# gmlwns2000/sea-attention

Hardware: AMD Instinct MI355X
Metric: tokens/sec + achieved HBM GB/s, OPT-1.3B SEA T=4096 k=64, 1/2/4/8 MI355X (higher is better)
Workload: dtype bf16

## Files before the change

include/sea_hip.h:

```cpp
#ifndef SEA_HIP_H
#define SEA_HIP_H

#include <stdint.h>

#ifdef __cplusplus
extern "C" {
#endif

#define SEA_ABI_VERSION 6

enum sea_dtype { SEA_F32 = 0, SEA_F16 = 1, SEA_BF16 = 2 };

enum sea_error {
  SEA_OK = 0,
  SEA_EINVAL = -1,
  SEA_EUNSUPPORTED = -2,
  SEA_ELAUNCH = -3
};

typedef void* sea_stream_t;

int sea_version(void);
const char* sea_last_error(void);

// ... 42 lines not shown

int sea_csr_elmul(const float* in_values, float* out_values,
                  const void* other, int dtype, const int64_t* other_strides ,
                  int64_t N, int64_t H, int64_t T_dst, int64_t T_src,
                  const void* crow, const void* col, int idx_bytes, int64_t col_stride_n,
                  sea_stream_t stream);

int sea_csr_spmm(const float* values, const void* v, int dtype,
                 int64_t N, int64_t H, int64_t T_dst, int64_t T_src, int64_t D,
                 const int64_t* v_strides ,
                 const void* crow, const void* col, int idx_bytes, int64_t col_stride_n,
                 const int32_t* head_off,
                 float* out, sea_stream_t stream);

enum sea_attn_path { SEA_ATTN_AUTO = 0, SEA_ATTN_GATHER = 1, SEA_ATTN_TILE = 2, SEA_ATTN_KEYRANGE = 3 };
enum { SEA_ATTN_ROW_POOL_SHIFT = 4 };
int sea_sparse_attention(const void* q, const void* k, const void* v, int dtype,
                         int64_t N, int64_t H, int64_t T_dst, int64_t T_src, int64_t D,
                         const int64_t* q_strides, const int64_t* k_strides, const int64_t* v_strides,
                         const int32_t* crow, const int32_t* col, int64_t col_stride_n,
                         const int32_t* head_off,
                         const float* row_scale,
                         const void* avg, const int64_t* avg_strides,
                         const float* mix,
                         void* out, int out_dtype, const int64_t* out_strides,
                         float* probs_out, int64_t probs_stride_n,
                         const uint8_t* block_path,
                         int flags,
                         const uint32_t* bits, int64_t T_m, int is_causal, int max_k, int write_cols,
                         const int32_t* t_src_dev,
                         int64_t t_src_stride,
// ... 120 lines not shown
```

sea-attention_amd/_lib.py:

```python
import ctypes
import os
from ctypes import c_int, c_int32, c_int64, c_void_p, c_char_p, POINTER

import torch

from . import _build

SEA_F32, SEA_F16, SEA_BF16 = 0, 1, 2
ABI_VERSION = 6
_DTYPES = {torch.float32: SEA_F32, torch.float16: SEA_F16, torch.bfloat16: SEA_BF16}

_lib = None

i64 = c_int64
ptr = c_void_p
_i64p = POINTER(c_int64)

_SIGNATURES = {
    "sea_version": ([], c_int),
    "sea_last_error": ([], c_char_p),
    "sea_topk_select": ([ptr, c_int, i64, i64, i64, i64, i64, i64, i64, ptr, i64, i64, c_int, c_int,
                         ptr, ptr, ptr, ptr, ptr], c_int),
    "sea_mask_to_bits": ([ptr, c_int, i64, i64, i64, i64, i64, i64, i64, i64, c_int, c_int,
                          ptr, ptr, ptr, ptr], c_int),
# ... 47 lines not shown
                                ptr, i64, ptr, i64, i64, ptr, i64, ptr, i64, ptr, ptr, ptr, i64, c_int32, c_int32, c_int32, ptr],
                               c_int),
    "sea_performer_avg_supported": ([i64, i64, c_int], c_int),
    "sea_performer_plan": ([i64, i64, i64, i64, i64, c_int, _i64p, _i64p], c_int),
}

EXPORTED_SYMBOLS = tuple(_SIGNATURES)


def library_path():
    return _build.LIB_PATH


SEA_ATTN_AUTO, SEA_ATTN_GATHER, SEA_ATTN_TILE, SEA_ATTN_KEYRANGE = 0, 1, 2, 3
SEA_ATTN_ROW_POOL_SHIFT = 4
SEA_OK, SEA_EINVAL, SEA_EUNSUPPORTED = 0, -1, -2


def load(build_if_missing=True):
    global _lib
    if _lib is not None:
        return _lib
    override = os.environ.get("SEA_HIP_LIB")
    if override:
        if not os.path.exists(override):
            raise RuntimeError(f"SEA_HIP_LIB={override} does not exist")
        path = override
    else:
        path = _build.LIB_PATH
        if _build.is_stale():
# ... 92 lines not shown
```

sea-attention_amd/csrc/sea_attn.hip:

```cpp
#include "sea_attn.hpp"

namespace sea {

template <typename T, typename TO, int LPR, int U, bool WP>
__global__ __launch_bounds__(256) void sparse_attn_kernel(AttnParams p) {
  constexpr int VEC = Elem<T>::VEC;
  constexpr int KPI = 64 / LPR;
  int pair, tb;
  if (!map_block(p.N * p.H, p.TB, &pair, &tb)) return;
  const int n = pair / p.H, h = pair - n * p.H;
  const int t = tb * 4 + (threadIdx.x >> 6);
  if (t >= p.T_dst) return;
  if (kernel_is_idle(p)) return;
  const int lane = threadIdx.x & 63;
  const int grp = lane / LPR, sub = lane - grp * LPR;
  const bool dact = sub * VEC < p.D;

  const T* qp = reinterpret_cast<const T*>(p.q) + n * p.qs[0] + h * p.qs[1] + t * p.qs[2] + sub * VEC;
  const T* kb = reinterpret_cast<const T*>(p.k) + n * p.ks[0] + h * p.ks[1] + sub * VEC;
  const T* vb = reinterpret_cast<const T*>(p.v) + n * p.vs[0] + h * p.vs[1] + sub * VEC;

  uint4 qraw = make_uint4(0, 0, 0, 0);
  if (dact) qraw = *reinterpret_cast<const uint4*>(qp);
  const int row_beg = p.crow[(int64_t)n * (p.T_dst + 1) + t];
// ... 238 lines not shown
  return col[ec];
}

constexpr int SEA_ATTN_WARM_ROWS = 8;

template <typename T, typename TO, int LPR, int U, bool WP, int NWB, bool FUSE, bool DEC, bool ORD, bool X80>
__device__ __forceinline__ void attn_rows_body(const AttnParams& p) {
  static_assert(!DEC || FUSE, "the decode form is a fused form");
  static_assert(!ORD || (FUSE && !DEC && !WP), "rows are dealt from pools in the fused inference form only");
  static_assert(!X80 || LPR == 8, "d = 80: eight lanes per row");
  using F = RowFrag<T, X80>;
  constexpr int VEC = F::VEC, NF = F::NF;
  constexpr int RPW = 64 / LPR;
  constexpr int RPB = NWB * RPW;
  int pair, tb;
  if (kernel_is_idle(p) || !map_block(p.N * p.H, p.TB, &pair, &tb)) return;
  const int n = pair / p.H;
  const int h = (pair - n * p.H + n) % p.H;
  const int lane = threadIdx.x & 63;
  const int grp = lane / LPR, sub = lane - grp * LPR;
  const int gi = (int)(threadIdx.x >> 6) * RPW + grp;
  bool rowok;
  int t;
  if constexpr (ORD) {
    if (!pooled_row<LPR, RPB>(p, n, h, tb, grp, &t, &rowok)) return;
  } else {
    t = tb * RPB + rows_by_length<LPR, RPB>(slot_length(p, n, h, tb * RPB + gi), gi, sub, &rowok);
  }
  const bool dact = X80 || sub * VEC < p.D;
  const int tt = t < p.T_dst ? t : p.T_dst - 1;
  const int sube = dact ? sub : 0;
// ... 86 lines not shown
        }
        softmax_step<U>(s, mnew, vr, m, l, acc);
      }
    }
  }

  const int64_t ridx = ((int64_t)n * p.H + h) * p.T_dst + t;
  if (WP && rowok) {
    const float c = attn_row_factor(p, ridx, l);
    float* pr = p.probs + n * p.probs_stride_n;
    for (int e = beg + sub; e < end; e += LPR) pr[e] = __expf(pr[e] - m) * c;
  }
  if (rowok && dact) attn_epilogue<T, TO, X80>(p, ridx, n, h, t, sub, l, acc);
}

template <typename T, typename TO, int LPR, int U, bool WP, int NWB = 4, bool FUSE = false, bool DEC = false, bool ORD = false>
__global__ __launch_bounds__(NWB * 64, (FUSE && !DEC && sizeof(T) == 2 && !WP) ? 8 : 1) void sparse_attn_rows_kernel(AttnParams p) {
  attn_rows_body<T, TO, LPR, U, WP, NWB, FUSE, DEC, ORD, false>(p);
}

template <typename T, typename TO, int U, bool WP, int NWB = 4, bool FUSE = false, bool DEC = false, bool ORD = false>
__global__ __launch_bounds__(NWB * 64) void sparse_attn_rows80_kernel(AttnParams p) {
  attn_rows_body<T, TO, 8, U, WP, NWB, FUSE, DEC, ORD, true>(p);
}

template <int LPR, bool X80>
struct Decode1Lds {
  static constexpr int CH = LPR == 8 ? 256 : 128;
  static constexpr int DL = LPR * (8 + (X80 ? 2 : 0));
  static constexpr int bytes = CH * 8 + CH + CH * DL * 2;
};

template <typename T, typename TO, int LPR, bool X80 = false, bool PAGED = false, bool WP = false>
// ... 481 lines not shown
    const int64_t pool = 1ll << pool_log2;
    SEA_REQUIRE(pool <= 1024, SEA_EUNSUPPORTED, "%s: %s takes pools of at most 1024 rows (got %lld)", nm, rp, (long long)pool);
    const int64_t rpb = (dtype == SEA_F32 ? D > 32 : (D > 64 && D != 80)) ? 32 : 64;
    SEA_REQUIRE(pool % rpb == 0, SEA_EUNSUPPORTED, "%s: %s needs a pool that is a multiple of the %lld rows of a workgroup (got %lld)",
                nm, rp, (long long)rpb, (long long)pool);
    const int64_t pools = (T_dst + pool - 1) / pool, need = H * pools * pool;
    SEA_REQUIRE(block_path != nullptr && aligned16(block_path) && probs_stride_n >= need, SEA_EINVAL,
                "%s: %s needs a 16-byte aligned uint16 workspace in block_path with probs_stride_n >= %lld elements per batch "
                "item (got %lld)", nm, rp, (long long)need, (long long)probs_stride_n);
    order = reinterpret_cast<const uint16_t*>(block_path);
    order_stride_n = probs_stride_n;
    block_path = nullptr;
    probs_stride_n = 0;
  }
  const bool keyrange = (flags & 0xff) == SEA_ATTN_KEYRANGE;
  KeyRangeParams kr = {nullptr, 0, 0, 0};
  if (keyrange) {
    SEA_REQUIRE(bits != nullptr, SEA_EUNSUPPORTED, "%s: the key-range form is a fused form (bits is NULL)", nm);
    SEA_REQUIRE(t_src_dev == nullptr && block_table == nullptr && t_src_stride == 0, SEA_EUNSUPPORTED,
                "%s: the key-range form has no decode or paged form (t_src_dev / block_table)", nm);
    SEA_REQUIRE(write_cols == 0, SEA_EUNSUPPORTED, "%s: the key-range form writes no columns (write_cols must be 0)", nm);
    SEA_REQUIRE(N > 0 && H > 0 && T_dst > 0 && T_src > 0 && D > 0, SEA_EINVAL, "%s: bad shape", nm);
    SEA_REQUIRE(dtype == SEA_F32 ? (D == 32 || D == 64) : (D == 64 || D == 128), SEA_EUNSUPPORTED,
                "%s: the key-range form takes 16-bit D in {64, 128} or fp32 D in {32, 64} (dtype %d, D=%lld)", nm, dtype, (long long)D);
    const int64_t rk = (flags >> 16) & 0x7fff;
    SEA_REQUIRE(rk > 0, SEA_EINVAL, "%s: the key-range form needs range_keys (1 .. 32767) in bits 16..30 of flags", nm);
    const int64_t nr = (T_src + rk - 1) / rk;
    SEA_REQUIRE(nr <= 64, SEA_EUNSUPPORTED, "%s: the key-range form takes at most 64 ranges (%lld keys in ranges of %lld: %lld)", nm,
                (long long)T_src, (long long)rk, (long long)nr);
    SEA_REQUIRE(block_path == nullptr, SEA_EINVAL, "%s: the key-range form takes no plan (block_path must be NULL)", nm);
// ... 59 lines not shown
  p.probs = probs_out; p.probs_stride_n = probs_stride_n;
  p.sel = nullptr; p.sel_want = 0; p.TB16 = (int)((T_dst + 15) / 16);
  p.sel_count = nullptr; p.sel_total = (int)(N * H * p.TB16);
  p.sel_num = D >= 128 ? 13 : 1; p.sel_den = D >= 128 ? 20 : 2;
  p.bits = bits; p.col_w = const_cast<int32_t*>(col); p.T_m = (int)T_m; p.W = (int)((H * T_m + 31) / 32);
  p.max_k = max_k; p.is_causal = is_causal;
  p.fuse_cap = 8192;
  p.write_cols = write_cols != 0;
  p.t_src_dev = t_src_dev;
  SEA_REQUIRE(t_src_stride >= 0 && t_src_stride * N < (1ll << 31), SEA_EINVAL, "%s: bad T_src stride %lld", nm,
              (long long)t_src_stride);
  p.t_src_stride = (int)t_src_stride;
  p.table = block_table; p.table_stride = (int)table_stride; p.page_shift = block_table ? __builtin_ctzll(page_rows) : 0;
  p.order = order; p.order_stride_n = order_stride_n;
  p.pool_rows = order ? 1 << pool_log2 : 0; p.pools = order ? (int)((T_dst + p.pool_rows - 1) / p.pool_rows) : 0;
  if (t_src_dev) {
    SEA_REQUIRE(bits != nullptr && T_dst <= SEA_ATTN_WARM_ROWS, SEA_EUNSUPPORTED,
                "%s: the decode form takes T_dst <= %d rows per sequence", nm, SEA_ATTN_WARM_ROWS);
    SEA_REQUIRE(probs_out == nullptr || probs_stride_n >= col_stride_n, SEA_EINVAL,
                "%s: the decode form's probs_out needs probs_stride_n >= col_stride_n (%lld < %lld)", nm,
                (long long)probs_stride_n, (long long)col_stride_n);
  }
  if (bits) {
    SEA_REQUIRE(path != SEA_ATTN_TILE && block_path == nullptr, SEA_EUNSUPPORTED, "%s: the fused interpolation runs on the gather kernels", nm);
    SEA_REQUIRE(T_m > 0 && T_m % 32 == 0 && max_k > 0, SEA_EUNSUPPORTED, "%s: fused interpolation needs T_m %% 32 == 0", nm);
    if (t_src_dev) SEA_REQUIRE(H * T_src < (1ll << 31), SEA_EUNSUPPORTED, "%s: the decode form needs int32 ids (H*T_cap < 2^31)", nm);
    else SEA_REQUIRE(H * T_src < (1ll << 24), SEA_EUNSUPPORTED, "%s: H*T_src must stay below 2^24 (fp32-exact ids)", nm);
  }
  p.TB = (int)((T_dst + 3) / 4);
  hipStream_t s = (hipStream_t)stream;
// ... 20 lines not shown
    p.sel_want = 1;
    rc = launch_attn_tile(p, dtype, out_dtype, flags, s);
    SEA_REQUIRE(rc == SEA_OK, rc, "%s: tile kernel launch parameters rejected (flags 0x%x)", nm, flags);
    SEA_CHECK_LAUNCH(nm);
    p.sel_want = 0;
  }
  if (dtype == SEA_F32) rc = launch_attn<float, float>(p, s);
  else if (dtype == SEA_F16) rc = out_dtype == SEA_F32 ? launch_attn<__half, float>(p, s) : launch_attn<__half, __half>(p, s);
  else rc = out_dtype == SEA_F32 ? launch_attn<__hip_bfloat16, float>(p, s) : launch_attn<__hip_bfloat16, __hip_bfloat16>(p, s);
  SEA_REQUIRE(rc == SEA_OK, rc, "%s: unsupported head size %lld", nm, (long long)D);
  SEA_CHECK_LAUNCH(nm);
  return SEA_OK;
}

extern "C" int64_t sea_attention_few_rows(void) { return SEA_ATTN_FEW_ROWS; }

extern "C" int sea_attention_plan(const uint32_t* bits, int64_t N, int64_t H, int64_t T_dst, int64_t T_src, int64_t T_m,
                                  int is_causal, float entries_per_tile, uint8_t* block_path, sea_stream_t stream) {
  const char* nm = "sea_attention_plan";
  SEA_REQUIRE(bits && block_path, SEA_EINVAL, "%s: null pointer", nm);
  SEA_REQUIRE(N > 0 && H > 0 && T_dst > 0 && T_src > 0 && T_m > 0, SEA_EINVAL, "%s: bad shape", nm);
  SEA_REQUIRE(hipMemsetAsync(block_path + plan_count_offset(N, H, (T_dst + 15) / 16), 0, 4, (hipStream_t)stream) == hipSuccess,
              SEA_ELAUNCH, "%s: memset failed", nm);
  const int rc = launch_attn_plan(bits, (int)N, (int)H, (int)T_dst, (int)T_src, (int)T_m, is_causal,
                                  entries_per_tile > 0.f ? entries_per_tile : 30.0f, block_path, (hipStream_t)stream);
  SEA_REQUIRE(rc == SEA_OK, rc, "%s: needs T_m %% 32 == 0, H <= 64 and H * T_m <= 32768", nm);
  SEA_CHECK_LAUNCH(nm);
  return SEA_OK;
}

// ... 70 lines not shown
```

sea-attention_amd/csrc/sea_attn.hpp:

```cpp
#pragma once
#include "sea_common.hpp"

namespace sea {

struct AttnParams {
  const void *q, *k, *v;
  int64_t qs[3], ks[3], vs[3];
  int N, H, T_dst, T_src, D;
  const int32_t* crow;
  const int32_t* col;
  int64_t col_stride_n;
  const int32_t* head_off;
  const float* row_scale;
  const void* avg;
  int64_t as[3];
  const float* mix;
  void* out;
  int64_t os[3];
  float* probs;
  int64_t probs_stride_n;
  const uint8_t* sel;
  int sel_want, TB16;
  const int32_t* sel_count;
  int sel_total, sel_num, sel_den;
  int TB;
  const uint32_t* bits;
  int32_t* col_w;
  int T_m, W, max_k, is_causal, fuse_cap;
  int write_cols;
  const int32_t* t_src_dev;
  int t_src_stride;
  const int32_t* table;
  int table_stride, page_shift;
  const uint16_t* order;
  int64_t order_stride_n;
  int pool_rows, pools;
};

template <typename TO, int VEC> __device__ inline void store_frag(TO* dst, const float* f);
template <> __device__ inline void store_frag<float, 4>(float* dst, const float* f) {
  *reinterpret_cast<float4*>(dst) = make_float4(f[0], f[1], f[2], f[3]);
}
template <> __device__ inline void store_frag<float, 8>(float* dst, const float* f) {
  *reinterpret_cast<float4*>(dst) = make_float4(f[0], f[1], f[2], f[3]);
  *reinterpret_cast<float4*>(dst + 4) = make_float4(f[4], f[5], f[6], f[7]);
}
template <> __device__ inline void store_frag<__hip_bfloat16, 8>(__hip_bfloat16* dst, const float* f) {
  union { uint4 u; __hip_bfloat16 h[8]; } r;
#pragma unroll
  for (int i = 0; i < 8; ++i) r.h[i] = __float2bfloat16(f[i]);
  *reinterpret_cast<uint4*>(dst) = r.u;
// ... 5 lines not shown
  *reinterpret_cast<uint4*>(dst) = r.u;
}
template <> __device__ inline void store_frag<__hip_bfloat16, 4>(__hip_bfloat16* dst, const float* f) {
  union { uint2 u; __hip_bfloat16 h[4]; } r;
#pragma unroll
  for (int i = 0; i < 4; ++i) r.h[i] = __float2bfloat16(f[i]);
  *reinterpret_cast<uint2*>(dst) = r.u;
}
template <> __device__ inline void store_frag<__half, 4>(__half* dst, const float* f) {
  union { uint2 u; __half h[4]; } r;
#pragma unroll
  for (int i = 0; i < 4; ++i) r.h[i] = __float2half(f[i]);
  *reinterpret_cast<uint2*>(dst) = r.u;
}

__device__ inline bool map_block(int NH, int TB, int* pair, int* tb) {
  const int bid = blockIdx.x;
  const int xcd = bid & 7, slot = bid >> 3;
  const int pl = slot / TB;
  const int full = NH >> 3;
  if (pl < full) {
    *tb = slot - pl * TB;
    *pair = pl * 8 + xcd;
    return true;
  }
  const int r = NH - full * 8;
  const int item = (slot - pl * TB) * 8 + xcd;
  if (pl > full || item >= r * TB) return false;
  const int pr = item / TB;
  *tb = item - pr * TB;
  *pair = full * 8 + pr;
  return true;
}

template <int CTRL> __device__ inline float dpp_f(float x) {
  return __int_as_float(__builtin_amdgcn_update_dpp(0, __float_as_int(x), CTRL, 0xF, 0xF, true));
}

template <int LPR> __device__ inline float group_sum(float x) {
  if (LPR >= 2) x += dpp_f<0xB1>(x);
  if (LPR >= 4) x += dpp_f<0x4E>(x);
  if (LPR >= 8) x += dpp_f<0x141>(x);
  if (LPR >= 16) x += dpp_f<0x140>(x);
  if (LPR >= 32) x += __shfl_xor(x, 16);
  if (LPR >= 64) x += __shfl_xor(x, 32);
  return x;
}
// ... 195 lines not shown
```

sea-attention_amd/csrc/sea_attn_tile.hip:

```cpp
#include "sea_attn.hpp"
#include <type_traits>

namespace sea {

typedef __attribute__((ext_vector_type(8))) __bf16 at_bf8;
typedef __attribute__((ext_vector_type(8))) _Float16 at_h8;
typedef __attribute__((ext_vector_type(2))) __bf16 at_bf2;
typedef __attribute__((ext_vector_type(2))) _Float16 at_h2;
typedef __attribute__((ext_vector_type(2))) float at_f2;
typedef __attribute__((ext_vector_type(4))) float at_f4;
typedef __attribute__((ext_vector_type(4))) short at_s4;

template <typename T> struct TileT;
template <> struct TileT<__hip_bfloat16> {
  static constexpr bool SPLIT = true;
  __device__ static inline at_f4 mfma(const uint4& a, const uint4& b, at_f4 c) {
    return __builtin_amdgcn_mfma_f32_16x16x32_bf16(__builtin_bit_cast(at_bf8, a), __builtin_bit_cast(at_bf8, b), c, 0, 0, 0);
  }
  __device__ static inline uint32_t pack(float a, float b) {
    const at_f2 f = {a, b};
    return __builtin_bit_cast(uint32_t, __builtin_convertvector(f, at_bf2));
  }
  __device__ static inline float lo_val(uint32_t pk) { return __uint_as_float(pk << 16); }
  __device__ static inline float hi_val(uint32_t pk) { return __uint_as_float(pk & 0xffff0000u); }
// ... 52 lines not shown
}
template <> __device__ inline void unpack4<__half>(const uint2& r, float* f) {
  const float2 a = __half22float2(__builtin_bit_cast(__half2, r.x)), b = __half22float2(__builtin_bit_cast(__half2, r.y));
  f[0] = a.x; f[1] = a.y; f[2] = b.x; f[3] = b.y;
}

template <typename T, typename TO, int D, int RT, int NW>
__global__ __launch_bounds__(NW * 64) void sparse_attn_tile_kernel(AttnParams p, int KW, int wave_lds) {
  using G = TileGeom<D>;
  using X = TileT<T>;
  constexpr int ROWS = 16 * RT, KK = G::KK, MT = G::MT, CH = G::CH, VST = G::VST, VLD = G::VLD;
  constexpr bool SPLIT = X::SPLIT;
  constexpr float LOG2E = 1.4426950408889634f;
  extern __shared__ __attribute__((aligned(16))) char at_smem[];
  int pair, tb;
  if (kernel_is_idle(p) || !map_block(p.N * p.H, p.TB, &pair, &tb)) return;
  const int n = pair / p.H, h = pair - n * p.H;
  const int lane = threadIdx.x & 63, li = lane & 15, g = lane >> 4;
  const int wave = __builtin_amdgcn_readfirstlane((int)(threadIdx.x >> 6));
  const int t0 = (tb * NW + wave) * ROWS;
  if (t0 >= p.T_dst) return;

  const int WPR = KW >> 5, BST = WPR + 1;
  char* wbase = at_smem + wave * wave_lds;
  uint32_t* bm = reinterpret_cast<uint32_t*>(wbase);
  unsigned short* tl = reinterpret_cast<unsigned short*>(bm + ROWS * BST);
  char* vs = wbase + ((ROWS * BST * 4 + (KW / 16) * 2 + 15) & ~15);

  const char* kbase = reinterpret_cast<const char*>(reinterpret_cast<const T*>(p.k) + n * p.ks[0] + h * p.ks[1]);
  const char* vbase = reinterpret_cast<const char*>(reinterpret_cast<const T*>(p.v) + n * p.vs[0] + h * p.vs[1]);
  const uint32_t kst = (uint32_t)p.ks[2] * 2u, vst = (uint32_t)p.vs[2] * 2u;
// ... 370 lines not shown
```

sea-attention_amd/perlin_attention/attention.py:

```python
import math
import os
import warnings
from typing import NamedTuple, Optional

import torch
import torch.nn.functional as F
from torch import nn

from ..utils import get_bench
from .config import PerlinAttentionConfig, get_default_config
from .modules import CausalConv2d, KeepRes, UpsampleFP32
from .performer import FastAttention, ProjectionUpdater
from . import ops

timer = lambda name: get_bench().region(name)
mem = lambda name: get_bench().mem_region(name)
_C8_DECLINED = set()
ATTENTION_ROW_POOL: Optional[int] = 512
ATTENTION_ROW_POOL_HEAD_SIZES = (64, 128)


def _safe_to(t, d):
    return t.to(d) if isinstance(t, torch.Tensor) else t


class PerlinAttentionOutput(NamedTuple):
    loss: torch.Tensor
    context_layer: torch.Tensor
    partial_attention_probs: torch.Tensor
    partial_attention_mask: torch.Tensor
    estimated_attention_probs_m: torch.Tensor
    estimated_attention_probs: torch.Tensor
    dense_attention_probs: torch.Tensor
    key_for_score: torch.Tensor
# ... 58 lines not shown
        self.attention_head_size = int(config.hidden_size / config.num_attention_heads)
        self.all_head_size = self.num_attention_heads * self.attention_head_size
        self._warning_messages = ""

        self.benchmarking = False
        self.context_layer_dtype = None
        self.assume_not_padded = None
        self.materialize_csr = False
        self.return_attention_probs = False
        self.lazy_attention_probs = True
        self.lazy_csr_columns = True
        self.conv_z_epilogue = False
        self.sparse_kernel = "auto"
        self.key_range: Optional[int] = None
        self.attention_row_pool: Optional[int] = ATTENTION_ROW_POOL
        self.performer_segments = None
        self.force_torch_estimator = False
        self.dense_head_chunk = None
        self._fused_gates = None
        self._fused_selection = None
        self._avg_ahead = None

        d, H = self.attention_head_size, self.num_attention_heads
        pc = self.pconfig

        self.performer_nb_features = int(d * math.log(d) / pc.performer_nb_factor)
        self.performer = FastAttention(dim_heads=d, nb_features=self.performer_nb_features,
                                       causal=pc.causal, generalized_attention=pc.causal)
        self.performer_proj_updater = ProjectionUpdater(self.performer, 1000)
        if pc.attention_predictor_backend != 'performer':
# ... 726 lines not shown
                    plan = None
                    if (self.sparse_kernel == "auto" and not want_probs and qs.dtype != torch.float32
                            and HID in (64, 80, 128) and not csr.col_is_pending):
                        plan = ops.attention_plan(csr, T_M, is_causal=True)
                    if (self.key_range is not None and not want_probs and csr.col_is_pending and self.lazy_csr_columns
                            and T_SRC > self.key_range
                            and ops.keyrange_supported(qs.dtype, HID, T_M, T_SRC, int(self.key_range))):
                        res = ops.sparse_attention(qs, ks, vs, csr, row_scale=row_scale, avg=average_context_layer,
                                                   mix=average_scale, out=ctx.view(N, T, H, HID).permute(0, 2, 1, 3),
                                                   path="keyrange", range_keys=int(self.key_range))
                    else:
                        row_pool = self.attention_row_pool
                        if row_pool is not None and not (qs.dtype != torch.float32 and HID in ATTENTION_ROW_POOL_HEAD_SIZES
                                                         and ops.row_pool_supported(qs.dtype, HID, int(row_pool))):
                            row_pool = None
                        res = ops.sparse_attention(qs, ks, vs, csr, row_scale=row_scale, avg=average_context_layer,
                                                   mix=average_scale, out=ctx.view(N, T, H, HID).permute(0, 2, 1, 3),
                                                   want_probs=want_probs, path="gather" if want_probs else self.sparse_kernel,
                                                   plan=plan, keep_columns_pending=self.lazy_csr_columns and not want_probs,
                                                   row_pool=row_pool)
                    if want_probs:
                        probs_csr = csr.with_values(res[1])
        if probs_csr is not None:
            bench.register_temp_buffer('partial_attention_probs', None, lazy=lambda: ops.flat_csr_to_dense(probs_csr, T_SRC, H))
        if self.materialize_csr:
            return ctx, (probs_csr.to_sparse_csr() if probs_csr is not None else None), csr.to_sparse_csr()
        return ctx, probs_csr, csr

    def _forward_dense(self, q, v, q_for_score, k_for_score, t_attention_predictor, probs, causal_attention_mask,
                       dst_attention_mask, attention_scores_truth, FP_MIN, T_SRC, T_M, resize_dense, head_chunk=None):
        bench = get_bench()
        N, H, T, HID = q.shape
        k_, os_ = self.pconfig.k, self.pconfig.k_oversample
        loss = 0
        with timer("mask"):
# ... 96 lines not shown
```

sea-attention_amd/perlin_attention/ops/__init__.py:

```python
from .resize_dense import resize_from_m_to_t
from .flat_csr import resize_from_m_to_t_csr
from .flat_csr import flat_csr_elmul
from .flat_csr import flat_csr_masked_bmm
from .flat_csr import flat_csr_sdbmm
from .flat_csr import flat_csr_softmax
from .flat_csr import flat_csr_to_dense
from .flat_csr import (FlatCSR, fused_interp_supported, attention_few_rows, topk_to_csr, topk_mask, sparse_attention, sparse_attention_bytes, attention_plan, plan_blocks, make_plan,
                       sparse_attention_autograd, keyrange_supported, keyrange_workspace_floats,
                       row_pool_supported, row_pool_workspace, row_pool_workspace_elems,
                       keep_table_causal, keep_table_kernel_test, z_capacity, csr_from_selection)
from .predictor import (split_layernorm, predictor_tail, cumavg, performer_value, performer_supported, performer_avg_supported,
                        performer_step, performer_plan, performer_chunk_rows,
                        split_layernorm_c8, causal_conv_c8, causal_conv_c8_z, conv_z_supported, conv_c8_f32_supported, predictor_tail_z, pack_conv_weight, to_c8, from_c8,
                        predictor_mlp, predictor_mlp_supported, predictor_tail_select,
                        predictor_tail_select_supported, clear_prep_cache, prep_generation, pinned_prep, LazyTensor, realize,
                        decode_stage, c8_window_shift, decode_fork, decode_fork_staging_bytes, decode_cnn_tail_select, decode_cnn_supported, decode_cnn_emits, decode_tail_select_supported, DECODE_PREDICTOR_LENGTHS,
                        decode_gather_rows, decode_append_rows)
```

sea-attention_amd/perlin_attention/ops/flat_csr.py:

```python
import math
from ctypes import c_void_p, c_int64
from typing import Optional

import torch

from ... import _lib


def _p(t: Optional[torch.Tensor]):
    return c_void_p(t.data_ptr()) if t is not None else c_void_p(0)


class FlatCSR:

    def __init__(self, crow, col, head_off, H, T_src, bits=None, row_nnz=None, vals=None):
        self.crow, self._col, self.head_off = crow, col, head_off
        self.H, self.T_src = H, T_src
        self.bits, self.row_nnz = bits, row_nnz
        self.vals = vals
        self.N, self.T_dst = crow.shape[0], crow.shape[1] - 1
        self._wire = None
        self._pending = None
        self.t_src_dev = None

# ... 221 lines not shown
def keyrange_workspace_floats(N: int, H: int, T_dst: int, D: int, n_ranges: int) -> int:
    return N * H * n_ranges * T_dst * (D + 2)


ROW_POOL_MAX = 1024


def row_pool_supported(dtype, D: int, row_pool: int) -> bool:
    vec = 4 if dtype == torch.float32 else 8
    rpb = 64 if (D == 80 and vec == 8) or D <= 8 * vec else 32
    return row_pool >= rpb and row_pool <= ROW_POOL_MAX and row_pool & (row_pool - 1) == 0


def row_pool_workspace_elems(N: int, H: int, T_dst: int, row_pool: int) -> int:
    return N * H * -(-T_dst // row_pool) * row_pool


_BWD_WS = {}
_KEYRANGE_WS = {}
_ROW_POOL_WS = {}


def row_pool_workspace(N: int, H: int, T_dst: int, row_pool: int, device) -> torch.Tensor:
    per = row_pool_workspace_elems(1, H, T_dst, row_pool)
    return _stream_workspace(_ROW_POOL_WS, N * per * 2, device).view(torch.int16).view(N, H, per // H)


def _keyrange_workspace(N: int, stride: int, device) -> torch.Tensor:
    return _stream_workspace(_KEYRANGE_WS, N * stride * 4, device).view(torch.float32).view(N, stride)

# ... 83 lines not shown
    _lib.require_gpu(csr.bits)
    nb = csr.N * csr.H * ((csr.T_dst + 15) // 16)
    buf = torch.empty((((nb + 3) & ~3) + 4,), dtype=torch.uint8, device=csr.bits.device)
    _lib.check(lib.sea_attention_plan(_p(csr.bits), csr.N, csr.H, csr.T_dst, csr.T_src, int(T_m), int(is_causal),
                                      float(entries_per_tile), _p(buf), _lib.stream_ptr()), "sea_attention_plan")
    return buf


@_lib.device_guarded
def sparse_attention(q, k, v, csr: FlatCSR, row_scale: Optional[torch.Tensor] = None,
                     avg: Optional[torch.Tensor] = None, mix: Optional[torch.Tensor] = None,
                     out: Optional[torch.Tensor] = None, out_dtype: Optional[torch.dtype] = None,
                     path: str = "auto", want_probs: bool = False, row_tiles: int = 0, key_window: int = 0,
                     plan: Optional[torch.Tensor] = None, fuse_emit: bool = True, keep_columns_pending: bool = False,
                     block_table: Optional[torch.Tensor] = None, range_keys: Optional[int] = None,
                     row_pool: Optional[int] = None, probs_out: Optional[torch.Tensor] = None):
    lib = _lib.load()
    if row_pool is not None and not row_pool_supported(q.dtype, q.shape[-1], int(row_pool)):
        raise ValueError(f"sparse_attention(row_pool={row_pool}): a power of two up to {ROW_POOL_MAX} and a multiple of the rows a "
                         f"workgroup walks (64 for rows of 8 lanes, 32 for rows of 16; got {q.dtype}, d = {q.shape[-1]})")
    want_probs = want_probs or probs_out is not None
    if probs_out is not None:
        _lib.require_gpu(probs_out)
        assert (probs_out.dtype == torch.float32 and probs_out.dim() == 2 and probs_out.shape[0] == csr.N
                and probs_out.shape[1] >= csr._col.shape[1] and probs_out.stride(1) == 1
                and (csr.N == 1 or probs_out.stride(0) >= csr._col.stride(0))), "probs_out: fp32 (N, >= z_cap), feature stride 1"
    _lib.require_gpu(q, k, v, csr.crow, block_table)
    keyrange = path == "keyrange"
    if keyrange:
        why = None
        if range_keys is None or not 1 <= int(range_keys) <= 32767:
            why = f"range_keys must be 1 .. 32767 (got {range_keys})"
# ... 66 lines not shown

    if keyrange:
        T_m_, max_k_, causal_, _emit = csr._pending
        n_ranges = -(-T_src // int(range_keys))
        stride = (keyrange_workspace_floats(1, H, T_dst, D, n_ranges) + 3) & ~3
        ws = _keyrange_workspace(N, stride, q.device)
        _lib.check(launch(csr._col, ws, None, _lib.SEA_ATTN_KEYRANGE | (int(range_keys) << 16), csr.bits, T_m_, int(causal_),
                          max_k_, 0), "sea_sparse_attention")
        return out
    if fused:
        T_m_, max_k_, causal_, _emit = csr._pending
        raw_col = csr._col
        probs = probs_out
        if want_probs and probs is None:
            probs = torch.zeros(raw_col.shape, dtype=torch.float32, device=q.device)
        flags, order = _lib.SEA_ATTN_GATHER, None
        if row_pool is not None and not (decode_form or paged or want_probs):
            flags |= (int(row_pool).bit_length() - 1) << _lib.SEA_ATTN_ROW_POOL_SHIFT
            order = row_pool_workspace(N, H, T_dst, int(row_pool), q.device)
        rc = launch(raw_col, probs, None, flags, csr.bits, T_m_, int(causal_), max_k_,
                    0 if keep_columns_pending else 1, csr.t_src_dev, order)
        if rc == 0:
            if not keep_columns_pending:
                csr._pending = None
            return (out, probs) if want_probs else out
        if rc != _lib.SEA_EUNSUPPORTED or paged:
            _lib.check(rc, "sea_sparse_attention")
    probs = probs_out
    if want_probs and probs is None:
        probs = torch.zeros(csr.col.shape, dtype=torch.float32, device=q.device)
    flags = _PATHS[path] | ((int(row_tiles) & 0xf) << 8)
    if key_window:
        assert key_window & (key_window - 1) == 0, "key_window is a power of two"
        flags |= (int(key_window).bit_length() - 1) << 12
    block_path = plan if (plan is not None and path == "auto" and not want_probs) else None
    _lib.check(launch(csr.col, probs, block_path, flags), "sea_sparse_attention")
    return (out, probs) if want_probs else out


def plan_blocks(plan: torch.Tensor, N: int, H: int, T_dst: int) -> torch.Tensor:
    tb = (T_dst + 15) // 16
    return plan[:N * H * tb].view(N, H, tb)


def make_plan(blocks: torch.Tensor) -> torch.Tensor:
    nb = blocks.numel()
# ... 162 lines not shown
```

Baseline: 15.66 million.

## Add heavy-first and grouped grid orders for sparse attention block scheduling

Extends the block-to-(pair,row-block) mapping with two new orders. Heavy-first walks causal row blocks from the last (longest) to the first to reduce tail imbalance. Grouped interleaves a few head pairs per XCD so their K/V stay resident in L2. A Python heuristic picks the order automatically from the K/V bytes per pair, and an optional timestamp probe is compiled under SEA_STAMP. The added index math is small, but grouping may cost locality or balance when the L2 estimate is wrong.

```diff
diff --git a/include/sea_hip.h b/include/sea_hip.h
--- a/include/sea_hip.h
+++ b/include/sea_hip.h
@@ -80,7 +80,7 @@
                  float* out, sea_stream_t stream);
 
 enum sea_attn_path { SEA_ATTN_AUTO = 0, SEA_ATTN_GATHER = 1, SEA_ATTN_TILE = 2, SEA_ATTN_KEYRANGE = 3 };
-enum { SEA_ATTN_ROW_POOL_SHIFT = 4 };
+enum { SEA_ATTN_ROW_POOL_SHIFT = 4, SEA_ATTN_GRID_ORDER_SHIFT = 16, SEA_ATTN_GRID_GROUP_SHIFT = 18 };
 int sea_sparse_attention(const void* q, const void* k, const void* v, int dtype,
                          int64_t N, int64_t H, int64_t T_dst, int64_t T_src, int64_t D,
                          const int64_t* q_strides, const int64_t* k_strides, const int64_t* v_strides,
diff --git a/sea-attention_amd/_lib.py b/sea-attention_amd/_lib.py
--- a/sea-attention_amd/_lib.py
+++ b/sea-attention_amd/_lib.py
@@ -85,6 +85,7 @@
 
 SEA_ATTN_AUTO, SEA_ATTN_GATHER, SEA_ATTN_TILE, SEA_ATTN_KEYRANGE = 0, 1, 2, 3
 SEA_ATTN_ROW_POOL_SHIFT = 4
+SEA_ATTN_GRID_ORDER_SHIFT, SEA_ATTN_GRID_GROUP_SHIFT = 16, 18
 SEA_OK, SEA_EINVAL, SEA_EUNSUPPORTED = 0, -1, -2
 
 
diff --git a/sea-attention_amd/csrc/sea_attn.hip b/sea-attention_amd/csrc/sea_attn.hip
--- a/sea-attention_amd/csrc/sea_attn.hip
+++ b/sea-attention_amd/csrc/sea_attn.hip
@@ -7,7 +7,7 @@
   constexpr int VEC = Elem<T>::VEC;
   constexpr int KPI = 64 / LPR;
   int pair, tb;
-  if (!map_block(p.N * p.H, p.TB, &pair, &tb)) return;
+  if (!map_block((int)blockIdx.x, p.N * p.H, p.TB, p.grid_order, p.grid_group, &pair, &tb)) return;
   const int n = pair / p.H, h = pair - n * p.H;
   const int t = tb * 4 + (threadIdx.x >> 6);
   if (t >= p.T_dst) return;
@@ -276,7 +276,10 @@
   constexpr int RPW = 64 / LPR;
   constexpr int RPB = NWB * RPW;
   int pair, tb;
-  if (kernel_is_idle(p) || !map_block(p.N * p.H, p.TB, &pair, &tb)) return;
+  constexpr bool ORDERED = FUSE && !DEC;
+  if (kernel_is_idle(p) ||
+      !map_block((int)blockIdx.x, p.N * p.H, p.TB, ORDERED ? p.grid_order : (int)SEA_GRID_ASCENDING, ORDERED ? p.grid_group : 1, &pair, &tb))
+    return;
   const int n = pair / p.H;
   const int h = (pair - n * p.H + n) % p.H;
   const int lane = threadIdx.x & 63;
@@ -393,9 +396,30 @@
   if (rowok && dact) attn_epilogue<T, TO, X80>(p, ridx, n, h, t, sub, l, acc);
 }
 
+#ifdef SEA_STAMP
+constexpr int SEA_ATTN_STAMP_BLOCKS = 1 << 16;
+__device__ unsigned long long sea_attn_grid_stamps[3 * SEA_ATTN_STAMP_BLOCKS];
+#define ATTN_GRID_STAMP(i)                                                                                     \
+  do {                                                                                                         \
+    if (threadIdx.x == 0 && blockIdx.x < (unsigned)SEA_ATTN_STAMP_BLOCKS)                                      \
+      sea_attn_grid_stamps[3 * blockIdx.x + (i)] = __builtin_amdgcn_s_memrealtime();                           \
+  } while (0)
+#define ATTN_GRID_STAMP_XCC()                                                                                  \
+  do {                                                                                                         \
+    if (threadIdx.x == 0 && blockIdx.x < (unsigned)SEA_ATTN_STAMP_BLOCKS)                                      \
+      sea_attn_grid_stamps[3 * blockIdx.x + 2] = __builtin_amdgcn_s_getreg(20 | (3 << 11)) & 0xf;  \
+  } while (0)
+#else
+#define ATTN_GRID_STAMP(i) do {} while (0)
+#define ATTN_GRID_STAMP_XCC() do {} while (0)
+#endif
+
 template <typename T, typename TO, int LPR, int U, bool WP, int NWB = 4, bool FUSE = false, bool DEC = false, bool ORD = false>
 __global__ __launch_bounds__(NWB * 64, (FUSE && !DEC && sizeof(T) == 2 && !WP) ? 8 : 1) void sparse_attn_rows_kernel(AttnParams p) {
+  ATTN_GRID_STAMP(0);
+  ATTN_GRID_STAMP_XCC();
   attn_rows_body<T, TO, LPR, U, WP, NWB, FUSE, DEC, ORD, false>(p);
+  ATTN_GRID_STAMP(1);
 }
 
 template <typename T, typename TO, int U, bool WP, int NWB = 4, bool FUSE = false, bool DEC = false, bool ORD = false>
@@ -907,6 +931,14 @@
     probs_stride_n = 0;
   }
   const bool keyrange = (flags & 0xff) == SEA_ATTN_KEYRANGE;
+  int grid_order = SEA_GRID_ASCENDING, grid_group = 1;
+  if (!keyrange) {
+    grid_order = (flags >> SEA_ATTN_GRID_ORDER_SHIFT) & 3;
+    grid_group = 1 << ((flags >> SEA_ATTN_GRID_GROUP_SHIFT) & 3);
+    flags &= 0xffff;
+    SEA_REQUIRE(grid_order <= SEA_GRID_GROUPED && grid_group <= 4, SEA_EINVAL,
+                "%s: grid order %d with groups of %d pairs: orders 0 .. 2, groups of 1, 2 or 4", nm, grid_order, grid_group);
+  }
   KeyRangeParams kr = {nullptr, 0, 0, 0};
   if (keyrange) {
     SEA_REQUIRE(bits != nullptr, SEA_EUNSUPPORTED, "%s: the key-range form is a fused form (bits is NULL)", nm);
@@ -996,6 +1028,9 @@
   p.table = block_table; p.table_stride = (int)table_stride; p.page_shift = block_table ? __builtin_ctzll(page_rows) : 0;
   p.order = order; p.order_stride_n = order_stride_n;
   p.pool_rows = order ? 1 << pool_log2 : 0; p.pools = order ? (int)((T_dst + p.pool_rows - 1) / p.pool_rows) : 0;
+  const bool prefill = t_src_dev == nullptr && N * H * T_dst > SEA_ATTN_FEW_ROWS;
+  p.grid_order = prefill ? grid_order : (int)SEA_GRID_ASCENDING;
+  p.grid_group = prefill ? grid_group : 1;
   if (t_src_dev) {
     SEA_REQUIRE(bits != nullptr && T_dst <= SEA_ATTN_WARM_ROWS, SEA_EUNSUPPORTED,
                 "%s: the decode form takes T_dst <= %d rows per sequence", nm, SEA_ATTN_WARM_ROWS);
@@ -1046,6 +1081,33 @@
 }
 
 extern "C" int64_t sea_attention_few_rows(void) { return SEA_ATTN_FEW_ROWS; }
+
+extern "C" int64_t sea_attention_grid_map(int64_t NH, int64_t TB, int order, int group, int32_t* pair, int32_t* tb, int32_t* has_work) {
+  const char* nm = "sea_attention_grid_map";
+  SEA_REQUIRE(pair && tb && has_work, SEA_EINVAL, "%s: null pointer", nm);
+  SEA_REQUIRE(NH > 0 && TB > 0 && 8 * ((NH + 7) / 8) * TB < (1ll << 31), SEA_EINVAL, "%s: bad grid %lld x %lld", nm, (long long)NH, (long long)TB);
+  SEA_REQUIRE(order >= 0 && order <= SEA_GRID_GROUPED && (group == 1 || group == 2 || group == 4), SEA_EINVAL,
+              "%s: grid order %d with groups of %d pairs: orders 0 .. 2, groups of 1, 2 or 4", nm, order, group);
+  const int64_t blocks = 8 * ((NH + 7) / 8) * TB;
+  for (int64_t b = 0; b < blocks; ++b) {
+    int pr = -1, rb = -1;
+    has_work[b] = map_block((int)b, (int)NH, (int)TB, order, group, &pr, &rb) ? 1 : 0;
+    pair[b] = pr;
+    tb[b] = rb;
+  }
+  return blocks;
+}
+
+#ifdef SEA_STAMP
+extern "C" int sea_debug_attn_grid_stamps(unsigned long long* host, int64_t blocks) {
+  if (blocks > SEA_ATTN_STAMP_BLOCKS) return SEA_EINVAL;
+  const size_t bytes = sizeof(unsigned long long) * 3 * (size_t)blocks;
+  if (hipMemcpyFromSymbol(host, HIP_SYMBOL(sea_attn_grid_stamps), bytes) != hipSuccess) return SEA_ELAUNCH;
+  void* dev = nullptr;
+  if (hipGetSymbolAddress(&dev, HIP_SYMBOL(sea_attn_grid_stamps)) != hipSuccess || hipMemset(dev, 0, bytes) != hipSuccess) return SEA_ELAUNCH;
+  return SEA_OK;
+}
+#endif
 
 extern "C" int sea_attention_plan(const uint32_t* bits, int64_t N, int64_t H, int64_t T_dst, int64_t T_src, int64_t T_m,
                                   int is_causal, float entries_per_tile, uint8_t* block_path, sea_stream_t stream) {
diff --git a/sea-attention_amd/csrc/sea_attn.hpp b/sea-attention_amd/csrc/sea_attn.hpp
--- a/sea-attention_amd/csrc/sea_attn.hpp
+++ b/sea-attention_amd/csrc/sea_attn.hpp
@@ -35,6 +35,7 @@
   const uint16_t* order;
   int64_t order_stride_n;
   int pool_rows, pools;
+  int grid_order, grid_group;
 };
 
 template <typename TO, int VEC> __device__ inline void store_frag(TO* dst, const float* f);
@@ -70,23 +71,35 @@
   *reinterpret_cast<uint2*>(dst) = r.u;
 }
 
-__device__ inline bool map_block(int NH, int TB, int* pair, int* tb) {
-  const int bid = blockIdx.x;
+enum { SEA_GRID_ASCENDING = 0, SEA_GRID_HEAVY_FIRST = 1, SEA_GRID_GROUPED = 2 };
+__host__ __device__ inline bool map_block(int bid, int NH, int TB, int order, int G, int* pair, int* tb) {
   const int xcd = bid & 7, slot = bid >> 3;
-  const int pl = slot / TB;
   const int full = NH >> 3;
-  if (pl < full) {
-    *tb = slot - pl * TB;
-    *pair = pl * 8 + xcd;
+  const bool desc = order != SEA_GRID_ASCENDING;
+  if (slot < full * TB) {
+    if (order != SEA_GRID_GROUPED || G == 1) {
+      const int pl = slot / TB, rb = slot - pl * TB;
+      *tb = desc ? TB - 1 - rb : rb;
+      *pair = pl * 8 + xcd;
+      return true;
+    }
+    const int grp = slot / (G * TB), w = slot - grp * (G * TB);
+    const int left = full - grp * G, cnt = left < G ? left : G;
+    const int rb = w / cnt;
+    *tb = TB - 1 - rb;
+    *pair = (grp * G + (w - rb * cnt)) * 8 + xcd;
     return true;
   }
   const int r = NH - full * 8;
-  const int item = (slot - pl * TB) * 8 + xcd;
-  if (pl > full || item >= r * TB) return false;
-  const int pr = item / TB;
-  *tb = item - pr * TB;
+  const int item = (slot - full * TB) * 8 + xcd;
+  if (item >= r * TB) return false;
+  const int pr = item / TB, rb = item - pr * TB;
+  *tb = desc ? TB - 1 - rb : rb;
   *pair = full * 8 + pr;
   return true;
+}
+__device__ inline bool map_block(int NH, int TB, int* pair, int* tb) {
+  return map_block((int)blockIdx.x, NH, TB, SEA_GRID_ASCENDING, 1, pair, tb);
 }
 
 template <int CTRL> __device__ inline float dpp_f(float x) {
diff --git a/sea-attention_amd/csrc/sea_attn_tile.hip b/sea-attention_amd/csrc/sea_attn_tile.hip
--- a/sea-attention_amd/csrc/sea_attn_tile.hip
+++ b/sea-attention_amd/csrc/sea_attn_tile.hip
@@ -90,7 +90,7 @@
   constexpr float LOG2E = 1.4426950408889634f;
   extern __shared__ __attribute__((aligned(16))) char at_smem[];
   int pair, tb;
-  if (kernel_is_idle(p) || !map_block(p.N * p.H, p.TB, &pair, &tb)) return;
+  if (kernel_is_idle(p) || !map_block((int)blockIdx.x, p.N * p.H, p.TB, p.grid_order, p.grid_group, &pair, &tb)) return;
   const int n = pair / p.H, h = pair - n * p.H;
   const int lane = threadIdx.x & 63, li = lane & 15, g = lane >> 4;
   const int wave = __builtin_amdgcn_readfirstlane((int)(threadIdx.x >> 6));
diff --git a/sea-attention_amd/perlin_attention/attention.py b/sea-attention_amd/perlin_attention/attention.py
--- a/sea-attention_amd/perlin_attention/attention.py
+++ b/sea-attention_amd/perlin_attention/attention.py
@@ -18,6 +18,7 @@
 _C8_DECLINED = set()
 ATTENTION_ROW_POOL: Optional[int] = 512
 ATTENTION_ROW_POOL_HEAD_SIZES = (64, 128)
+ATTENTION_GRID_ORDER = "auto"
 
 
 def _safe_to(t, d):
@@ -106,6 +107,7 @@
         self.sparse_kernel = "auto"
         self.key_range: Optional[int] = None
         self.attention_row_pool: Optional[int] = ATTENTION_ROW_POOL
+        self.attention_grid_order = ATTENTION_GRID_ORDER
         self.performer_segments = None
         self.force_torch_estimator = False
         self.dense_head_chunk = None
@@ -862,11 +864,14 @@
                         if row_pool is not None and not (qs.dtype != torch.float32 and HID in ATTENTION_ROW_POOL_HEAD_SIZES
                                                          and ops.row_pool_supported(qs.dtype, HID, int(row_pool))):
                             row_pool = None
+                        grid_order = self.attention_grid_order
+                        if grid_order == "auto":
+                            grid_order = ops.grid_order_default(qs.dtype, HID, T_SRC)
                         res = ops.sparse_attention(qs, ks, vs, csr, row_scale=row_scale, avg=average_context_layer,
                                                    mix=average_scale, out=ctx.view(N, T, H, HID).permute(0, 2, 1, 3),
                                                    want_probs=want_probs, path="gather" if want_probs else self.sparse_kernel,
                                                    plan=plan, keep_columns_pending=self.lazy_csr_columns and not want_probs,
-                                                   row_pool=row_pool)
+                                                   row_pool=row_pool, grid_order=grid_order)
                     if want_probs:
                         probs_csr = csr.with_values(res[1])
         if probs_csr is not None:
diff --git a/sea-attention_amd/perlin_attention/ops/__init__.py b/sea-attention_amd/perlin_attention/ops/__init__.py
--- a/sea-attention_amd/perlin_attention/ops/__init__.py
+++ b/sea-attention_amd/perlin_attention/ops/__init__.py
@@ -7,7 +7,7 @@
 from .flat_csr import flat_csr_to_dense
 from .flat_csr import (FlatCSR, fused_interp_supported, attention_few_rows, topk_to_csr, topk_mask, sparse_attention, sparse_attention_bytes, attention_plan, plan_blocks, make_plan,
                        sparse_attention_autograd, keyrange_supported, keyrange_workspace_floats,
-                       row_pool_supported, row_pool_workspace, row_pool_workspace_elems,
+                       row_pool_supported, row_pool_workspace, row_pool_workspace_elems, GRID_ORDERS, GRID_GROUPS, grid_group_rule, grid_order_default, attention_grid_map,
                        keep_table_causal, keep_table_kernel_test, z_capacity, csr_from_selection)
 from .predictor import (split_layernorm, predictor_tail, cumavg, performer_value, performer_supported, performer_avg_supported,
                         performer_step, performer_plan, performer_chunk_rows,
diff --git a/sea-attention_amd/perlin_attention/ops/flat_csr.py b/sea-attention_amd/perlin_attention/ops/flat_csr.py
--- a/sea-attention_amd/perlin_attention/ops/flat_csr.py
+++ b/sea-attention_amd/perlin_attention/ops/flat_csr.py
@@ -1,3 +1,4 @@
+import ctypes
 import math
 from ctypes import c_void_p, c_int64
 from typing import Optional
@@ -259,6 +260,51 @@
 
 def row_pool_workspace_elems(N: int, H: int, T_dst: int, row_pool: int) -> int:
     return N * H * -(-T_dst // row_pool) * row_pool
+
+
+GRID_ORDERS = ("ascending", "heavy-first", "grouped")
+GRID_GROUPS = (1, 2, 4)
+GRID_GROUP_L2_BYTES = 2 << 20
+
+
+def grid_group_rule(dtype, D: int, T_src: int) -> int:
+    pair_bytes = 2 * T_src * D * (4 if dtype == torch.float32 else 2)
+    return max([g for g in GRID_GROUPS if g * pair_bytes <= GRID_GROUP_L2_BYTES], default=1)
+
+
+def grid_order_default(dtype, D: int, T_src: int):
+    if dtype == torch.float32:
+        return None
+    pair_bytes = 2 * T_src * D * 2
+    if pair_bytes < (1 << 20) or pair_bytes > (4 << 20):
+        return None
+    return ("grouped", 2) if 2 * pair_bytes <= GRID_GROUP_L2_BYTES else "heavy-first"
+
+
+def _grid_order_flags(grid_order, dtype, D: int, T_src: int) -> int:
+    if grid_order is None:
+        return 0
+    name, group = grid_order if isinstance(grid_order, tuple) else (grid_order, None)
+    if name not in GRID_ORDERS or (group is not None and (name != "grouped" or group not in GRID_GROUPS)):
+        raise ValueError(f"sparse_attention(grid_order={grid_order!r}): one of {GRID_ORDERS}, or (\"grouped\", G) with G in {GRID_GROUPS}")
+    if name == "grouped" and group is None:
+        group = grid_group_rule(dtype, D, T_src)
+    return (GRID_ORDERS.index(name) << _lib.SEA_ATTN_GRID_ORDER_SHIFT) | \
+        ((int(group or 1).bit_length() - 1) << _lib.SEA_ATTN_GRID_GROUP_SHIFT)
+
+
+def attention_grid_map(NH: int, TB: int, grid_order="ascending", group: int = 1):
+    import numpy as np
+    lib = _lib.load()
+    fn = lib.sea_attention_grid_map
+    fn.argtypes, fn.restype = [ctypes.c_int64, ctypes.c_int64, ctypes.c_int, ctypes.c_int, ctypes.c_void_p, ctypes.c_void_p,
+                               ctypes.c_void_p], ctypes.c_int64
+    blocks = 8 * ((NH + 7) // 8) * TB
+    pair, tb, work = (np.empty(blocks, dtype=np.int32) for _ in range(3))
+    got = fn(NH, TB, GRID_ORDERS.index(grid_order), group, pair.ctypes.data, tb.ctypes.data, work.ctypes.data)
+    if got != blocks:
+        raise RuntimeError(f"sea_attention_grid_map({NH}, {TB}, {grid_order}, {group}) = {got}: {lib.sea_last_error().decode()}")
+    return pair, tb, work
 
 
 _BWD_WS = {}
@@ -372,8 +418,9 @@
                      path: str = "auto", want_probs: bool = False, row_tiles: int = 0, key_window: int = 0,
                      plan: Optional[torch.Tensor] = None, fuse_emit: bool = True, keep_columns_pending: bool = False,
                      block_table: Optional[torch.Tensor] = None, range_keys: Optional[int] = None,
-                     row_pool: Optional[int] = None, probs_out: Optional[torch.Tensor] = None):
-    lib = _lib.load()
+                     row_pool: Optional[int] = None, grid_order=None, probs_out: Optional[torch.Tensor] = None):
+    lib = _lib.load()
+    order_flags = _grid_order_flags(grid_order, q.dtype, q.shape[-1], csr.T_src)
     if row_pool is not None and not row_pool_supported(q.dtype, q.shape[-1], int(row_pool)):
         raise ValueError(f"sparse_attention(row_pool={row_pool}): a power of two up to {ROW_POOL_MAX} and a multiple of the rows a "
                          f"workgroup walks (64 for rows of 8 lanes, 32 for rows of 16; got {q.dtype}, d = {q.shape[-1]})")
@@ -470,7 +517,7 @@
         probs = probs_out
         if want_probs and probs is None:
             probs = torch.zeros(raw_col.shape, dtype=torch.float32, device=q.device)
-        flags, order = _lib.SEA_ATTN_GATHER, None
+        flags, order = _lib.SEA_ATTN_GATHER | (0 if decode_form or paged else order_flags), None
         if row_pool is not None and not (decode_form or paged or want_probs):
             flags |= (int(row_pool).bit_length() - 1) << _lib.SEA_ATTN_ROW_POOL_SHIFT
             order = row_pool_workspace(N, H, T_dst, int(row_pool), q.device)
@@ -485,7 +532,7 @@
     probs = probs_out
     if want_probs and probs is None:
         probs = torch.zeros(csr.col.shape, dtype=torch.float32, device=q.device)
-    flags = _PATHS[path] | ((int(row_tiles) & 0xf) << 8)
+    flags = _PATHS[path] | ((int(row_tiles) & 0xf) << 8) | (0 if decode_form else order_flags)
     if key_window:
         assert key_window & (key_window - 1) == 0, "key_window is a power of two"
         flags |= (int(key_window).bit_length() - 1) << 12
```

Measured after the change: 16.04 million (median of 6 runs). +2.5%, better.
